# ruolin/strawberry

Measured on AMD Instinct MI355X. Metric: loci/s, EM-to-convergence (+ FPKM/TPM epilogue), C3, higher is better.
Workload: dtype f64; 1 GPU; C3 human-scale synthetic: 60000 loci/GPU, niso~1+Geom(0.25), nrow~LogNormal(ln30,1), 2e8 fragments; loci_per_gpu=60000, fragments_per_gpu=200000086, collective=none (one rank), steps_pipelined=True

## Files before the change

### strawberry_amd/csrc/sbgpu_api.hip

```cpp
#include <hip/hip_runtime.h>

#include <cstdio>
#include <cstdlib>
#include <chrono>
#include <cmath>
#include <cstring>
#include <mutex>
#include <new>
#include <string>
#include <system_error>
#include <thread>
#include <vector>

#include "../../include/sbgpu.h"
#include "api_internal.h"
#include "binweight_device.h"
#include "em_device.h"
#include "em_wide.h"
#include "plan.h"

namespace {

thread_local std::string g_err;

int fail(int code, const std::string &msg)
{
   g_err = msg;
   return code;
}

#define HIP_TRY(expr)                                                                         \
   do {                                                                                       \
      hipError_t e_ = (expr);                                                                 \
      if (e_ != hipSuccess)                                                                   \
         return fail(SBGPU_EHIP, std::string(#expr) + ": " + hipGetErrorString(e_));          \
   } while (0)

constexpr int kAuxStreams = 8;
constexpr int kMaxPhaseEvents = 6;
constexpr int kKindStream[sb::kNumKinds] = {0, 0, 0, 2, 6, 1};

}

struct sbgpu_ctx {
   int device = 0;
   int n_cu = 256;
   hipDeviceProp_t prop;
   hipStream_t stream = nullptr;
   hipStream_t aux[kAuxStreams] = {};
   hipEvent_t fork = nullptr;
   hipEvent_t join[kAuxStreams] = {};
   unsigned split_runs = 0;
   int wave_alt = -1;
   hipEvent_t t0[sb::kNumKinds] = {}, t1[sb::kNumKinds] = {};
   hipEvent_t tp[kMaxPhaseEvents + 1] = {};
   bool timed[sb::kNumKinds] = {};
   bool timing = false;
   int n_phase_timed = 0;
   char *scratch[sb::kScratchSlots] = {};
   size_t scratch_bytes[sb::kScratchSlots] = {};
   int32_t *d_pdf_support = nullptr;
   int32_t *wide_error = nullptr;
   static constexpr int kMaxStages = 16;
   hipEvent_t stage_ev[kMaxStages][2] = {};
   const char *stage_name[kMaxStages] = {};
   int n_stages = 0;
   bool stage_open = false;
   char *pinned[4] = {};
   size_t pinned_bytes[4] = {};
   hipStream_t copy_stream = nullptr;
   hipEvent_t order_ev[6] = {};
   size_t pairs_hint = 0;
   sb::ResidentAnnotation *resident = nullptr;
   sb::ContextKeep context_keep;
   char *boot_scratch = nullptr;
   size_t boot_scratch_cap = 0;
   sb::BootKeep boot_keep;
   char *boot_result = nullptr;
   size_t boot_result_cap = 0;
};

namespace sb {
int api_fail(int code, const std::string &msg) { return fail(code, msg); }
hipStream_t ctx_stream(const sbgpu_ctx_t *ctx) { return ctx->stream; }
hipStream_t ctx_aux_stream(const sbgpu_ctx_t *ctx, int i) { return (i >= 0 && i < kAuxStreams) ? ctx->aux[i] : ctx->stream; }
int ctx_cu_count(const sbgpu_ctx_t *ctx) { return ctx->n_cu; }
int ctx_device(const sbgpu_ctx_t *ctx) { return ctx->device; }
void ctx_stage_reset(sbgpu_ctx_t *ctx) { ctx->n_stages = 0, ctx->stage_open = false; }
void ctx_stage_begin(sbgpu_ctx_t *ctx, const char *name, hipStream_t s)
{
   if (!ctx->timing || ctx->stage_open || ctx->n_stages >= sbgpu_ctx::kMaxStages) return;
   hipEvent_t *ev = ctx->stage_ev[ctx->n_stages];
   for (int i = 0; i < 2; ++i)
      if (!ev[i] && hipEventCreate(&ev[i]) != hipSuccess) return;
   if (hipEventRecord(ev[0], s) != hipSuccess) return;
   ctx->stage_name[ctx->n_stages] = name;
   ctx->stage_open = true;
}
void ctx_stage_end(sbgpu_ctx_t *ctx, hipStream_t s)
{
   if (!ctx->stage_open) return;
   (void)hipEventRecord(ctx->stage_ev[ctx->n_stages][1], s);
   ctx->stage_open = false;
   ++ctx->n_stages;
}
hipError_t ctx_pinned(sbgpu_ctx_t *ctx, int slot, size_t bytes, char **out)
{
   *out = nullptr;
   if (slot < 0 || slot >= 4) return hipErrorInvalidValue;
   if (bytes < 4096) bytes = 4096;
   if (ctx->pinned_bytes[slot] < bytes) {
      if (ctx->pinned[slot]) (void)hipHostFree(ctx->pinned[slot]);
      ctx->pinned[slot] = nullptr;
      ctx->pinned_bytes[slot] = 0;
      const size_t want = bytes + bytes / 4;
      hipError_t e = hipHostMalloc((void **)&ctx->pinned[slot], want, hipHostMallocDefault);
      if (e != hipSuccess) return e;
      ctx->pinned_bytes[slot] = want;
   }
   *out = ctx->pinned[slot];
   return hipSuccess;
}
hipError_t ctx_copy_stream(sbgpu_ctx_t *ctx, hipStream_t *out)
{
   if (!ctx->copy_stream) {
      hipError_t e = hipStreamCreateWithFlags(&ctx->copy_stream, hipStreamNonBlocking);
      if (e != hipSuccess) return e;
   }
   *out = ctx->copy_stream;
   return hipSuccess;
}
hipError_t ctx_event(sbgpu_ctx_t *ctx, int which, hipEvent_t *out)
{
   if (which < 0 || which >= 6) return hipErrorInvalidValue;
   if (!ctx->order_ev[which]) {
      hipError_t e = hipEventCreateWithFlags(&ctx->order_ev[which], hipEventDisableTiming);
      if (e != hipSuccess) return e;
   }
   *out = ctx->order_ev[which];
   return hipSuccess;
}
namespace {
struct DevBlock {
   char *p;
   size_t cap;
   int device;
};
struct DevPool {
   std::mutex m;
   std::vector<DevBlock> blocks;
   size_t bytes = 0;
   size_t limit = 0;
};
size_t dev_pool_limit(DevPool &pool)
{
   if (pool.limit) return pool.limit;
   size_t lim = (size_t)4 << 30;
   if (const char *e = std::getenv("SBGPU_POOL_GB")) {
      lim = (size_t)std::max(0.0, std::atof(e) * 1073741824.0);
   } else {
      size_t free_b = 0, total_b = 0;
      if (hipMemGetInfo(&free_b, &total_b) == hipSuccess && total_b / 2 > lim) lim = total_b / 2;
      else (void)hipGetLastError();
   }
   pool.limit = lim ? lim : 1;
   return pool.limit;
}
DevPool &dev_pool()
{
   static DevPool *p = new DevPool();
   return *p;
}
}
hipError_t dev_take(size_t bytes, char **out, size_t *capacity)
{
   *out = nullptr;
   *capacity = 0;
   if (bytes < 256) bytes = 256;
   int device = 0;
   hipError_t e = hipGetDevice(&device);
   if (e != hipSuccess) return e;
   DevPool &pool = dev_pool();
   {
      std::lock_guard<std::mutex> g(pool.m);
      size_t best = pool.blocks.size();
      for (size_t i = 0; i < pool.blocks.size(); ++i) {
         const DevBlock &b = pool.blocks[i];
         if (b.device == device && b.cap >= bytes && b.cap <= 2 * bytes + (1u << 20) && (best == pool.blocks.size() || b.cap < pool.blocks[best].cap)) best = i;
      }
      if (best < pool.blocks.size()) {
         *out = pool.blocks[best].p;
         *capacity = pool.blocks[best].cap;
         pool.bytes -= pool.blocks[best].cap;
         pool.blocks.erase(pool.blocks.begin() + (long)best);
         return hipSuccess;
      }
   }
   const size_t want = bytes + bytes / 16;
   e = hipMalloc(out, want);
   if (e != hipSuccess) {
      std::vector<DevBlock> idle;
      {
         std::lock_guard<std::mutex> g(pool.m);
         idle.swap(pool.blocks);
         pool.bytes = 0;
      }
      for (const DevBlock &b : idle) (void)hipFree(b.p);
      (void)hipGetLastError();
      e = hipMalloc(out, want);
      if (e != hipSuccess) return e;
   }
   *capacity = want;
   return hipSuccess;
}
size_t dev_release_idle()
{
   std::vector<DevBlock> idle;
   size_t bytes = 0;
   {
      DevPool &pool = dev_pool();
      std::lock_guard<std::mutex> g(pool.m);
      idle.swap(pool.blocks);
      bytes = pool.bytes;
      pool.bytes = 0;
   }
   for (const DevBlock &b : idle) (void)hipFree(b.p);
   return bytes;
}
namespace {
thread_local int g_give_without_device_sync = 0;
}
DevGiveStreamSynced::DevGiveStreamSynced() { ++g_give_without_device_sync; }
DevGiveStreamSynced::~DevGiveStreamSynced() { --g_give_without_device_sync; }
void dev_give(char *block, size_t capacity)
{
   if (!block) return;
   int current = 0, owner = -1;
   const bool have_current = hipGetDevice(&current) == hipSuccess;
// ... 188 lines not shown
            if (kb < 0) {
               k = 2;
            } else {
               kb = 1e3 / kb;
            }
         } else {
            kb = 1e3 / (double)len[u];
         }
         if (k != 2) {
            f = th[u] * rpm * kb;
            sum_fpkm += f;
         }
         fpkm[jb + u] = f;
         keep[jb + u] = k;
      }
   }
   double kept_sum = 0.0;
   for (int64_t jb = j0; jb < j1; jb += 4) {
      double f[4];
      int32_t kk[4];
#pragma unroll
      for (int u = 0; u < 4; ++u) {
         const bool in = jb + u < j1;
         f[u] = in ? fpkm[jb + u] : 0.0;
         kk[u] = in ? keep[jb + u] : 0;
      }
#pragma unroll
      for (int u = 0; u < 4; ++u) {
         if (jb + u >= j1) break;
         double fr = 0.0;
         int32_t k = kk[u];
         if (k != 2) fr = f[u] / sum_fpkm;
         if (p.filter_by_expression && fr < p.min_isoform_frac) k = 0;
         frac[jb + u] = fr;
         keep[jb + u] = k;
         if (k) kept_sum += f[u];
      }
   }
   return kept_sum;
}

__global__ __launch_bounds__(256) void abundance_kernel(int64_t n_loci, const int64_t *iso_off, const double *theta,
                                                        const int32_t *status, const int32_t *length,
                                                        sbgpu_abundance_params_t p, double *fpkm, double *frac,
                                                        int32_t *keep, double *block_sum, unsigned *ticket, double *total)
{
   const int64_t l = (int64_t)blockIdx.x * blockDim.x + threadIdx.x;
   __shared__ double part[256];
   __shared__ int s_last;
   part[threadIdx.x] = l < n_loci ? abundance_locus(l, iso_off, theta, status, length, p, fpkm, frac, keep) : 0.0;
   __syncthreads();
   for (int w = 128; w > 0; w >>= 1) {
      if ((int)threadIdx.x < w) part[threadIdx.x] += part[threadIdx.x + w];
      __syncthreads();
   }
   if (threadIdx.x == 0) {
      __hip_atomic_store(&block_sum[blockIdx.x], part[0], __ATOMIC_RELAXED, __HIP_MEMORY_SCOPE_AGENT);
      asm volatile("s_waitcnt vmcnt(0)" ::: "memory");
      const unsigned t = __hip_atomic_fetch_add(ticket, 1u, __ATOMIC_RELAXED, __HIP_MEMORY_SCOPE_AGENT);
      s_last = t == gridDim.x - 1;
   }
   __syncthreads();
   if (!s_last) return;
   double acc = 0.0;
   for (unsigned i = threadIdx.x; i < gridDim.x; i += 256)
      acc += __hip_atomic_load(&block_sum[i], __ATOMIC_RELAXED, __HIP_MEMORY_SCOPE_AGENT);
   part[threadIdx.x] = acc;
   __syncthreads();
   for (int w = 128; w > 0; w >>= 1) {
      if ((int)threadIdx.x < w) part[threadIdx.x] += part[threadIdx.x + w];
      __syncthreads();
   }
   if (threadIdx.x == 0) {
      *total = part[0];
      __hip_atomic_store(ticket, 0u, __ATOMIC_RELAXED, __HIP_MEMORY_SCOPE_AGENT);
   }
}

__global__ __launch_bounds__(1024) void sum_kernel(int64_t n, const double *x, double *out)
{
   __shared__ double s[1024];
   double acc = 0.0;
   for (int64_t i = threadIdx.x; i < n; i += 1024) acc += x[i];
   s[threadIdx.x] = acc;
   __syncthreads();
   for (int w = 512; w > 0; w >>= 1) {
      if ((int)threadIdx.x < w) s[threadIdx.x] += s[threadIdx.x + w];
      __syncthreads();
   }
   if (threadIdx.x == 0) *out = s[0];
}

__global__ void delay_kernel(unsigned long long ticks)
{
   const unsigned long long t0 = __builtin_amdgcn_s_memrealtime();
   while (__builtin_amdgcn_s_memrealtime() - t0 < ticks) __builtin_amdgcn_s_sleep(32);
}

__global__ void tpm_kernel(int64_t n, const double *fpkm, const int32_t *keep, const double *total,
                           double *tpm)
{
   const int64_t i = (int64_t)blockIdx.x * blockDim.x + threadIdx.x;
   if (i >= n) return;
   const double t = *total;
   tpm[i] = keep[i] ? 1e6 * fpkm[i] / t : 0.0;
}

}

extern "C" {

const char *sbgpu_version(void) { return "libsbgpu 0.1 (gfx950, strawberry EM hot path)"; }

#ifndef SBGPU_BUILD_ID
#define SBGPU_BUILD_ID "unknown"
#endif
const char *sbgpu_build_id(void) { return SBGPU_BUILD_ID; }

const char *sbgpu_last_error(void) { return g_err.c_str(); }

int sbgpu_device_count(void)
{
   int n = 0;
   if (hipGetDeviceCount(&n) != hipSuccess) return 0;
   return n;
}

int sbgpu_init(int device, sbgpu_ctx_t **ctx_out)
{
   if (!ctx_out) return fail(SBGPU_EINVAL, "sbgpu_init: null ctx_out");
   *ctx_out = nullptr;
   int n = 0;
   if (hipGetDeviceCount(&n) != hipSuccess || n <= 0) return fail(SBGPU_ENODEV, "sbgpu_init: no HIP device");
   if (device < 0 || device >= n) return fail(SBGPU_ENODEV, "sbgpu_init: device index out of range");
   HIP_TRY(hipSetDevice(device));
   sbgpu_ctx *c = new (std::nothrow) sbgpu_ctx();
   if (!c) return fail(SBGPU_ENOMEM, "sbgpu_init: out of host memory");
   c->device = device;
   hipError_t e = hipGetDeviceProperties(&c->prop, device);
   if (e != hipSuccess) {
      delete c;
      return fail(SBGPU_EHIP, std::string("hipGetDeviceProperties: ") + hipGetErrorString(e));
   }
   if (std::strncmp(c->prop.gcnArchName, "gfx950", 6) != 0) {
      std::string arch = c->prop.gcnArchName;
      delete c;
      return fail(SBGPU_ENODEV, "sbgpu_init: device is " + arch + ", libsbgpu is built for gfx950 only");
   }
   c->n_cu = c->prop.multiProcessorCount;
   e = hipStreamCreateWithFlags(&c->stream, hipStreamNonBlocking);
   int prio_least = 0, prio_greatest = 0;
   (void)hipDeviceGetStreamPriorityRange(&prio_least, &prio_greatest);
   const bool use_prio = !(sb::exp_env("SBGPU_STREAM_PRIORITY") && std::atoi(sb::exp_env("SBGPU_STREAM_PRIORITY")) == 0);
   for (int i = 0; e == hipSuccess && i < kAuxStreams; ++i) {
      const bool long_kind = i == kKindStream[sb::kNumKinds - 1] || i == kKindStream[sb::kNumKinds - 2] || i == kKindStream[sb::kNumKinds - 3];
      e = hipStreamCreateWithPriority(&c->aux[i], hipStreamNonBlocking, (use_prio && long_kind) ? prio_greatest : 0);
      if (e == hipSuccess) e = hipEventCreateWithFlags(&c->join[i], hipEventDisableTiming);
   }
   if (e == hipSuccess) e = hipEventCreateWithFlags(&c->fork, hipEventDisableTiming);
   if (e == hipSuccess) e = hipMalloc((void **)&c->d_pdf_support, 8 * sizeof(int32_t));
   if (e == hipSuccess) e = hipHostMalloc((void **)&c->wide_error, sizeof(int32_t), hipHostMallocDefault);
   if (e == hipSuccess) *c->wide_error = 0;
   for (int k = 0; e == hipSuccess && k < sb::kNumKinds; ++k) {
      e = hipEventCreate(&c->t0[k]);
      if (e == hipSuccess) e = hipEventCreate(&c->t1[k]);
   }
   for (int i = 0; e == hipSuccess && i <= kMaxPhaseEvents; ++i) e = hipEventCreate(&c->tp[i]);
   if (e != hipSuccess) {
      sbgpu_finalize(c);
      return fail(SBGPU_EHIP, std::string("sbgpu_init: stream/event creation: ") + hipGetErrorString(e));
   }
   *ctx_out = c;
   return SBGPU_OK;
}

int sbgpu_finalize(sbgpu_ctx_t *c)
{
   if (!c) return SBGPU_OK;
   (void)hipSetDevice(c->device);
   for (int i = 0; i < kAuxStreams; ++i) {
      if (c->aux[i]) (void)hipStreamDestroy(c->aux[i]);
      if (c->join[i]) (void)hipEventDestroy(c->join[i]);
   }
   if (c->fork) (void)hipEventDestroy(c->fork);
   for (int k = 0; k < sb::kNumKinds; ++k) {
      if (c->t0[k]) (void)hipEventDestroy(c->t0[k]);
      if (c->t1[k]) (void)hipEventDestroy(c->t1[k]);
   }
   for (int i = 0; i <= kMaxPhaseEvents; ++i)
      if (c->tp[i]) (void)hipEventDestroy(c->tp[i]);
   if (c->stream) (void)hipStreamDestroy(c->stream);
   if (c->wide_error) (void)hipHostFree(c->wide_error);
   for (auto &ev : c->stage_ev)
      for (hipEvent_t e : ev)
         if (e) (void)hipEventDestroy(e);
   if (c->d_pdf_support) (void)hipFree(c->d_pdf_support);
   for (int i = 0; i < sb::kScratchSlots; ++i)
      if (c->scratch[i]) (void)hipFree(c->scratch[i]);
   for (int i = 0; i < 4; ++i)
      if (c->pinned[i]) (void)hipHostFree(c->pinned[i]);
   for (hipEvent_t ev : c->order_ev)
      if (ev) (void)hipEventDestroy(ev);
   if (c->copy_stream) (void)hipStreamDestroy(c->copy_stream);
   sb::ctx_boot_release(c);
   sb::ctx_set_resident_annotation(c, nullptr);
   sb::dev_give(c->boot_scratch, c->boot_scratch_cap);
   delete c;
   return SBGPU_OK;
}

int sbgpu_device_info(sbgpu_ctx_t *c, int64_t out[8])
{
   if (!c || !out) return fail(SBGPU_EINVAL, "sbgpu_device_info: null argument");
   out[0] = c->prop.multiProcessorCount;
   out[1] = c->prop.warpSize;
   out[2] = (int64_t)c->prop.maxSharedMemoryPerMultiProcessor;
   out[3] = c->prop.clockRate;
   out[4] = (int64_t)(c->prop.totalGlobalMem >> 20);
   out[5] = out[6] = out[7] = 0;
   return SBGPU_OK;
}

int64_t sbgpu_release_idle_memory(void) { return (int64_t)sb::dev_release_idle(); }

int sbgpu_synchronize(sbgpu_ctx_t *c, void *stream)
{
   if (!c) return fail(SBGPU_EINVAL, "sbgpu_synchronize: null ctx");
   HIP_TRY(hipStreamSynchronize((hipStream_t)stream));
   if (c->wide_error && *c->wide_error) {
      *c->wide_error = 0;
      return fail(SBGPU_EHIP, "a barrier of the wide-locus EM kernel timed out: the loci it served have no result");
   }
   return SBGPU_OK;
}

int sbgpu_plan_destroy(sbgpu_plan_t *p)
{
   if (!p) return SBGPU_OK;
   if (p->ctx) (void)hipSetDevice(p->ctx->device);
   sb::dev_give(p->d_arena, p->arena_cap);
   if (p->graph_exec) (void)hipGraphExecDestroy(p->graph_exec);
   delete p;
   return SBGPU_OK;
}

int sbgpu_plan_create(sbgpu_ctx_t *c, int64_t n_loci, const int64_t *row_off, const int64_t *iso_off,
                      const int64_t *f_off, sbgpu_plan_t **plan_out)
{
   if (!c || !plan_out) return fail(SBGPU_EINVAL, "sbgpu_plan_create: null argument");
   *plan_out = nullptr;
   sbgpu_plan *p = new (std::nothrow) sbgpu_plan();
   if (!p) return fail(SBGPU_ENOMEM, "sbgpu_plan_create: out of host memory");
   p->ctx = c;
   const char *err = "";
   sb::PlanTuning tune;
   if (const char *e = sb::exp_env("SBGPU_WAVE_RMULT")) tune.wave_rmult = std::atoi(e);
   if (const char *e = sb::exp_env("SBGPU_MAX_WAVES")) tune.max_waves = std::atoll(e);
   if (const char *e = sb::exp_env("SBGPU_LIGHT_BLOCK")) tune.light_block = std::atoi(e) != 0;
   if (const char *e = sb::exp_env("SBGPU_ORDER")) tune.order_by_work = std::string(e) == "work";
   if (const char *e = sb::exp_env("SBGPU_CLASS_ORDER")) tune.classes_by_prediction = std::string(e) != "cost";
   auto parse_list = [](const char *ev, auto conv, auto *out) {
      std::string spec = ev;
      size_t pos = 0;
      while (pos < spec.size()) {
         size_t q = spec.find(',', pos);
         if (q == std::string::npos) q = spec.size();
         out->push_back(conv(spec.substr(pos, q - pos)));
         pos = q + 1;
      }
   };
   if (const char *e = sb::exp_env("SBGPU_PHASES")) {
      tune.phases_auto = false;
      parse_list(e, [](const std::string &t) { return std::atoi(t.c_str()); }, &tune.phase_limits);
   }
   if (const char *e = sb::exp_env("SBGPU_PHASE_LAMBDA"))
      parse_list(e, [](const std::string &t) { return (!t.empty() && (t[0] == 't' || t[0] == 'T')) ? -1.0 : std::atof(t.c_str()); }, &tune.phase_lambda);
   const bool timing = std::getenv("SBGPU_HOST_TIMING") != nullptr;
   auto now = []() { return std::chrono::duration<double>(std::chrono::steady_clock::now().time_since_epoch()).count(); };
   double t_stage = now();
   auto stage = [&](const char *name) {
      if (timing) {
         const double t = now();
         std::fprintf(stderr, "sbgpu_plan_create: %-12s %.2f ms\n", name, (t - t_stage) * 1e3);
         t_stage = t;
      }
   };
   int rc = sb::build_host_plan(n_loci, row_off, iso_off, f_off, c->n_cu, tune, &p->host, &err);
   stage("size classes");
   if (rc != SBGPU_OK) {
      delete p;
      return fail(rc, err);
   }
   if (n_loci > 0) p->h_row_off.assign(row_off, row_off + n_loci + 1), p->h_iso_off.assign(iso_off, iso_off + n_loci + 1);
   else p->h_row_off.assign(1, 0), p->h_iso_off.assign(1, 0);
   auto bail = [&](hipError_t e, const char *what) {
      sbgpu_plan_destroy(p);
      return fail(e == hipErrorOutOfMemory ? SBGPU_ENOMEM : SBGPU_EHIP, std::string(what) + ": " + hipGetErrorString(e));
   };
   hipError_t e = hipSetDevice(c->device);
   if (e != hipSuccess) return bail(e, "hipSetDevice");
   const size_t nb = (size_t)(n_loci + 1) * sizeof(int64_t);
   std::vector<sb::WideDesc> wide_table;
   size_t wide_buf_doubles = 0;
   for (sb::SizeClass &sc : p->host.classes) {
      if (sc.kind != sb::kStream) continue;
      std::vector<std::pair<int, int32_t>> wide;
      std::vector<int32_t> rest;
// ... 66 lines not shown
      for (int32_t cap : p->host.lat[0].capacity) n_phased += cap;
   auto up = [](size_t bytes) { return (bytes + 255) & ~(size_t)255; };
   size_t at = 0;
   const size_t o_row = at; at += up(nb);
   const size_t o_iso = at; at += up(nb);
   const size_t o_f = at; at += up(nb);
   const size_t o_loci = at; at += up((size_t)(n_loci + 1) * sizeof(int32_t));
   const size_t o_tab = at; at += up(ncls_alloc * sizeof(sb::ClassDesc));
   const size_t o_cn = at; at += up(ncls_alloc * sizeof(int32_t));
   const size_t o_wtab = at; at += up((wide_table.size() + 1) * sizeof(sb::WideDesc));
   std::vector<size_t> o_ltab(nlat), o_lroute(nlat), o_lcnt(nlat), o_ltot(nlat), o_llist(nlat);
   for (size_t i = 0; i < nlat; ++i) {
      o_ltab[i] = at; at += up((p->host.lat[i].classes.size() + 1) * sizeof(sb::ClassDesc));
      o_lroute[i] = at; at += up((size_t)(n_loci + 1) * sizeof(int32_t));
   }
   const size_t o_tick = at; at += up(sizeof(unsigned));
   const size_t staged = at;
   const size_t o_cur = at;
   for (size_t i = 0; i < nlat; ++i) {
      o_lcnt[i] = at; at += up((p->host.lat[i].classes.size() + 1) * sizeof(int32_t));
      o_ltot[i] = at; at += up(sizeof(int32_t));
   }
   p->zero_bytes = at - o_cur;
   for (size_t i = 0; i < nlat; ++i) {
      o_llist[i] = at; at += up((size_t)(n_phased + 1) * sizeof(int32_t));
   }
   const size_t o_keep = at; at += up((size_t)p->host.n_rows + 1);
   const size_t o_sum = at; at += up((size_t)(n_loci + 1) * sizeof(double));
   const size_t o_wbuf = at; at += up((wide_buf_doubles + 1) * sizeof(double));
   if ((e = sb::dev_take(at, &p->d_arena, &p->arena_cap)) != hipSuccess) return bail(e, "hipMalloc(plan arena)");
   stage("hipMalloc");
   p->d_row_off = (int64_t *)(p->d_arena + o_row);
   p->d_iso_off = (int64_t *)(p->d_arena + o_iso);
   p->d_f_off = (int64_t *)(p->d_arena + o_f);
   p->d_loci_all = (int32_t *)(p->d_arena + o_loci);
   p->d_tables = (sb::ClassDesc *)(p->d_arena + o_tab);
   p->d_class_n = (int32_t *)(p->d_arena + o_cn);
   p->d_zero = p->d_arena + o_cur;
   p->lat.resize(nlat);
   for (size_t i = 0; i < nlat; ++i) {
      sbgpu_plan::LatDev &ld = p->lat[i];
      const sb::LatPhase &lp = p->host.lat[i];
      ld.d_table = (sb::ClassDesc *)(p->d_arena + o_ltab[i]);
      ld.d_route = (int32_t *)(p->d_arena + o_lroute[i]);
      ld.d_counts = (int32_t *)(p->d_arena + o_lcnt[i]);
      ld.d_total = (int32_t *)(p->d_arena + o_ltot[i]);
      ld.d_lists = (int32_t *)(p->d_arena + o_llist[i]);
      ld.n_classes = (int)lp.classes.size();
      ld.it_limit = lp.it_limit;
      ld.repack = lp.repack;
      ld.grid = (int)std::min<int64_t>(std::max<int64_t>(lp.max_blocks, 1), 32768);
   }
   p->d_row_keep = (uint8_t *)(p->d_arena + o_keep);
   p->d_locus_sum = (double *)(p->d_arena + o_sum);
   p->d_epi_ticket = (unsigned *)(p->d_arena + o_tick);
   p->d_wide_table = (sb::WideDesc *)(p->d_arena + o_wtab);
   p->d_wide_bufs = (double *)(p->d_arena + o_wbuf);
   std::vector<char> stage_buf(staged, 0);
   if (n_loci > 0) {
      std::memcpy(stage_buf.data() + o_row, row_off, nb);
      std::memcpy(stage_buf.data() + o_iso, iso_off, nb);
      std::memcpy(stage_buf.data() + o_f, f_off, nb);
   }
   int32_t *h_loci = (int32_t *)(stage_buf.data() + o_loci);
   sb::ClassDesc *table = (sb::ClassDesc *)(stage_buf.data() + o_tab);
   int32_t *h_cn = (int32_t *)(stage_buf.data() + o_cn);
   if (!wide_table.empty()) std::memcpy(stage_buf.data() + o_wtab, wide_table.data(), wide_table.size() * sizeof(sb::WideDesc));
   for (size_t i = 0; i < nlat; ++i) {
      const sb::LatPhase &lp = p->host.lat[i];
      sb::ClassDesc *lt = (sb::ClassDesc *)(stage_buf.data() + o_ltab[i]);
      int32_t loff = 0;
      for (size_t ci = 0; ci < lp.classes.size(); ++ci) {
         const sb::SizeClass &sc = lp.classes[ci];
         lt[ci].block_begin = 0;
         lt[ci].n = lp.capacity[ci];
         lt[ci].loci_off = loff;
         lt[ci].shape = sc.layout | (sc.rmult << 8) | (sc.lbG << 16);
         loff += lp.capacity[ci];
      }
      std::memcpy(stage_buf.data() + o_lroute[i], lp.route.data(), lp.route.size() * sizeof(int32_t));
   }
   size_t off = 0;
   size_t max_stream_iso = 0;
   for (int k = 0; k < sb::kNumKinds; ++k) p->launches[k] = KindLaunch();
   for (size_t ci = 0; ci < ncls; ++ci) {
      const sb::SizeClass &sc = p->host.classes[ci];
      KindLaunch &kl = p->launches[sc.kind];
      if (kl.n_classes == 0) {
         kl.first_class = (int)ci;
         kl.d_table = p->d_tables + ci;
         kl.block_threads = sc.block_threads;
      }
      table[ci].block_begin = kl.n_blocks;
      table[ci].n = (int32_t)sc.loci.size();
      table[ci].loci_off = (int32_t)off;
      table[ci].shape = sc.layout | (sc.rmult << 8) | (sc.lbG << 16);
      h_cn[ci] = table[ci].n;
      kl.n_blocks += sc.n_blocks;
      kl.n_classes += 1;
      std::memcpy(h_loci + off, sc.loci.data(), sc.loci.size() * sizeof(int32_t));
      p->loci_off.push_back((int64_t)off);
      off += sc.loci.size();
      if (sc.kind == sb::kStream) {
         for (int32_t l : sc.loci) {
            size_t k = (size_t)(iso_off[l + 1] - iso_off[l]);
            if (k > max_stream_iso) max_stream_iso = k;
         }
      }
   }
   stage("staging");
   if ((e = hipMemcpy(p->d_arena, stage_buf.data(), staged, hipMemcpyHostToDevice)) != hipSuccess) return bail(e, "hipMemcpy(plan)");
   if (wide_buf_doubles && (e = hipMemset(p->d_wide_bufs, 0, wide_buf_doubles * sizeof(double))) != hipSuccess) return bail(e, "hipMemset(plan)");
   stage("upload");
   size_t npad = 1;
   while (npad < max_stream_iso && npad < 64) npad <<= 1;
   if (max_stream_iso > 64) npad = 64 * ((max_stream_iso + 63) / 64);
   p->stream_lds_bytes = (3 + sb::kStreamThreads / 64) * npad * sizeof(double);
   *plan_out = p;
   return SBGPU_OK;
}

int sbgpu_plan_info(const sbgpu_plan_t *p, int64_t out[8])
{
   if (!p || !out) return fail(SBGPU_EINVAL, "sbgpu_plan_info: null argument");
   out[0] = p->host.n_loci;
   out[1] = p->host.n_rows;
   out[2] = p->host.n_iso;
   out[3] = p->host.n_elem;
   out[4] = (int64_t)p->host.classes.size();
   out[5] = p->host.n_stream_loci;
   out[6] = p->host.algorithmic_bytes;
   out[7] = p->n_wide_loci;
   return SBGPU_OK;
}

int sbgpu_plan_classes(const sbgpu_plan_t *p, int64_t *out, int cap)
{
   if (!p) return fail(SBGPU_EINVAL, "sbgpu_plan_classes: null plan");
   int n = (int)p->host.classes.size();
   for (int i = 0; i < n && i < cap && out; ++i) {
      const sb::SizeClass &sc = p->host.classes[i];
      out[i * 6 + 0] = sc.kind;
      out[i * 6 + 1] = sc.CPL * sc.CL;
      out[i * 6 + 2] = sc.R;
      out[i * 6 + 3] = sc.G;
      out[i * 6 + 4] = (int64_t)sc.loci.size();
      out[i * 6 + 5] = (int64_t)sc.n_blocks * (sc.block_threads / 64);
   }
   return n;
}

}

static int find_wave_alt(sbgpu_ctx_t *c)
{
   const int used[3] = {kKindStream[sb::kWaveH], kKindStream[sb::kBlock], kKindStream[sb::kBlockTall]};
   const int cand[5] = {1, 3, 4, 5, 7};
   if (hipDeviceSynchronize() != hipSuccess) return 0;
   for (int pass = 0; pass < 2; ++pass)
      for (int ci = 0; ci < 5; ++ci) {
         const auto t0 = std::chrono::steady_clock::now();
         for (int u = 0; u < 3; ++u) hipLaunchKernelGGL(delay_kernel, dim3(1), dim3(64), 0, c->aux[used[u]], 200ull * 100ull);
         hipLaunchKernelGGL(delay_kernel, dim3(1), dim3(64), 0, c->aux[cand[ci]], 200ull * 100ull);
         if (hipDeviceSynchronize() != hipSuccess) return 0;
         const double us = std::chrono::duration<double, std::micro>(std::chrono::steady_clock::now() - t0).count();
         if (pass == 1 && us < 330.0) return cand[ci];
      }
   return 0;
}

static int em_run_impl(sbgpu_ctx_t *c, const sbgpu_plan_t *p, const int32_t *d_count, const void *d_F_any, void *d_theta_any,
                       int32_t *d_status, int32_t *d_iters, void *stream, const bool f32, const void *d_row_bias = nullptr,
                       const void *d_iso_bias = nullptr, void *join_stream = nullptr)
{
   if (!c || !p) return fail(SBGPU_EINVAL, "sbgpu_em_run_device: null ctx/plan");
   if (p->host.n_loci == 0) return SBGPU_OK;
   if (!d_theta_any || !d_status || !d_iters || (!d_count && p->host.n_rows) || (!d_F_any && p->host.n_elem))
      return fail(SBGPU_EINVAL, "sbgpu_em_run_device: null device pointer");
   if (f32 && (p->launches[sb::kStream].n_classes > 0 || p->launches[sb::kWaveH].n_classes > 0))
      return fail(SBGPU_EUNSUPPORTED, "sbgpu_em_run_device_f32: the fp32 variant covers loci of up to 64 isoforms in the tile kernels only");
   if ((d_row_bias != nullptr) != (d_iso_bias != nullptr)) return fail(SBGPU_EINVAL, "sbgpu_em_run_device_bias: both bias arrays or none");
   bool stream_fallback = false;
   if (p->launches[sb::kStream].n_classes > 0)
      stream_fallback = (int32_t)p->host.classes[p->launches[sb::kStream].first_class].loci.size() > p->n_wide_loci;
   if (d_row_bias && (stream_fallback || !p->lat.empty()))
      return fail(SBGPU_EUNSUPPORTED, "sbgpu_em_run_device_bias: the bias factors are applied at tile load (tile kernels and the wide-locus kernel: "
                                      "no locus on the streaming fallback, no phases)");
   hipStream_t main = (hipStream_t)stream;
   sb::EmArgs a;
   a.row_bias = f32 ? nullptr : (const double *)d_row_bias;
   a.iso_bias = f32 ? nullptr : (const double *)d_iso_bias;
   a.row_off = p->d_row_off;
   a.iso_off = p->d_iso_off;
   a.f_off = p->d_f_off;
   a.count = d_count;
   a.F = (const double *)d_F_any;
   a.theta = (double *)d_theta_any;
   a.status = d_status;
   a.iters = d_iters;
   sb::EmArgsT<float> a32;
   a32.row_off = a.row_off, a32.iso_off = a.iso_off, a32.f_off = a.f_off, a32.count = a.count;
   a32.F = (const float *)d_F_any, a32.theta = (float *)d_theta_any, a32.status = d_status, a32.iters = d_iters;
   a32.row_bias = f32 ? (const float *)d_row_bias : nullptr, a32.iso_bias = f32 ? (const float *)d_iso_bias : nullptr;
   if (join_stream && (p->zero_bytes || p->n_wide_desc))
      for (int k = 0; k < sb::kNumKinds; ++k)
         if (p->launches[k].n_classes > 0) HIP_TRY(hipStreamWaitEvent(main, c->join[k], 0));
   if (p->zero_bytes) HIP_TRY(hipMemsetAsync(p->d_zero, 0, p->zero_bytes, main));
   if (p->n_wide_desc) HIP_TRY(hipMemsetAsync(d_status, 0xFF, (size_t)p->host.n_loci * sizeof(int32_t), main));
   int kinds = 0;
   for (int k = 0; k < sb::kNumKinds; ++k) kinds += p->launches[k].n_classes > 0;
   const bool fork = kinds > 1;
   static const bool wave_on_main = sb::exp_env("SBGPU_WAVE_ON_MAIN") && std::atoi(sb::exp_env("SBGPU_WAVE_ON_MAIN")) != 0;
   if (join_stream && fork && c->wave_alt < 0) {
      const char *forced = sb::exp_env("SBGPU_WAVE_ALT");
      c->wave_alt = forced ? std::max(0, std::min(7, std::atoi(forced))) : find_wave_alt(c);
      if (std::getenv("SBGPU_HOST_TIMING"))
         std::fprintf(stderr, "[sbgpu] split runs: the wave kinds' second stream = %d (0: none)%s\n", c->wave_alt, forced ? " (SBGPU_WAVE_ALT)" : "");
   }
   const int wave_slot = (join_stream && fork && c->wave_alt > 0 && !p->zero_bytes && !p->n_wide_desc && (c->split_runs++ & 1)) ? c->wave_alt : 0;
   auto stream_of = [&](int k) -> hipStream_t {
      if (!fork || (wave_on_main && kKindStream[k] == 0)) return main;
      return c->aux[kKindStream[k] == 0 ? wave_slot : kKindStream[k]];
   };
   if (fork) {
      HIP_TRY(hipEventRecord(c->fork, main));
      for (int k = 0; k < sb::kNumKinds; ++k)
         if (p->launches[k].n_classes > 0 && stream_of(k) != main) HIP_TRY(hipStreamWaitEvent(stream_of(k), c->fork, 0));
   }
   for (int k = 0; k < sb::kNumKinds; ++k) c->timed[k] = false;
   c->n_phase_timed = 0;
   const bool timing = c->timing;
   const bool wide_last = fork && p->n_wide_desc > 0;
   for (int pass = 0; pass < 2; ++pass)
   for (int k = sb::kNumKinds - 1; k >= 0; --k) {
      const KindLaunch &kl = p->launches[k];
      if (kl.n_classes == 0) continue;
      if ((pass == 1) != (wide_last && k == sb::kStream)) continue;
      if (pass == 1) {
         for (int o = 0; o < sb::kNumKinds; ++o) {
            if (o == k || p->launches[o].n_classes == 0) continue;
            HIP_TRY(hipEventRecord(c->join[o], stream_of(o)));
            HIP_TRY(hipStreamWaitEvent(stream_of(k), c->join[o], 0));
         }
      }
      hipStream_t s = stream_of(k);
      static const int wave_delay_us = sb::exp_env("SBGPU_WAVE_DELAY_US") ? std::atoi(sb::exp_env("SBGPU_WAVE_DELAY_US")) : 5;
      static const int block_delay_us = sb::exp_env("SBGPU_BLOCK_DELAY_US") ? std::atoi(sb::exp_env("SBGPU_BLOCK_DELAY_US")) : 5;
      const bool tall_runs = p->launches[sb::kBlockTall].n_classes > 0;
      int hold_us = 0;
      if (fork && k == sb::kBlock && tall_runs) hold_us = block_delay_us;
      if (fork && kKindStream[k] == 0) hold_us = wave_delay_us + ((tall_runs && p->launches[sb::kBlock].n_classes > 0) ? block_delay_us : 0);
      if (join_stream && !(p->zero_bytes || p->n_wide_desc)) hold_us = 0;
      if (hold_us > 0) {
         hipLaunchKernelGGL(delay_kernel, dim3(1), dim3(64), 0, s, (unsigned long long)hold_us * 100ull);
         HIP_TRY(hipGetLastError());
      }
      if (timing) HIP_TRY(hipEventRecord(c->t0[k], s));
      if (k == sb::kStream) {
         if (p->n_wide_desc) {
            p->wide_epoch = (p->wide_epoch % 0x1FFFFFu) + 1;
            int32_t *d_err = nullptr;
            HIP_TRY(hipHostGetDevicePointer((void **)&d_err, c->wide_error, 0));
            for (const sbgpu_plan::WideRound &r : p->wide_rounds) {
               sb::WideArgs wa;
               wa.a = a;
               wa.table = p->d_wide_table + r.first_desc;
               wa.n_desc = r.n_desc;
               wa.bufs = p->d_wide_bufs;
               wa.epoch = p->wide_epoch;
               wa.error = d_err;
               HIP_TRY(sb::launch_wide(wa, r.n_blocks, r.lds_bytes, s));
            }
         }
         const int32_t n_all = (int32_t)p->host.classes[kl.first_class].loci.size();
         if (n_all > p->n_wide_loci) {
            sb::ClassArgs ca = {};
            ca.loci = p->d_loci_all + p->loci_off[kl.first_class] + p->n_wide_loci;
            ca.n = n_all - p->n_wide_loci;
            ca.batch = 0;
            HIP_TRY(sb::launch_stream(a, ca, p->d_row_keep, ca.n, p->stream_lds_bytes, s));
         }
      } else {
         const bool wave_kind = k == sb::kWaveH || k == sb::kWave1 || k == sb::kWave2;
         const bool phased = wave_kind && !p->lat.empty() && !f32;
         sb::FusedLaunch fl;
         fl.a = a;
         fl.ph.table = kl.d_table;
         fl.ph.n_classes = kl.n_classes;
         fl.ph.lists_in = p->d_loci_all;
         fl.ph.n_in = p->d_class_n + kl.first_class;
         fl.ph.n_batches = kl.n_blocks;
         fl.ph.total_blocks = nullptr;
         fl.ph.lists_out = phased ? p->lat[0].d_lists : nullptr;
         fl.ph.n_out = phased ? p->lat[0].d_counts : nullptr;
         fl.ph.route = phased ? p->lat[0].d_route : nullptr;
         fl.ph.next_table = phased ? p->lat[0].d_table : nullptr;
         fl.ph.it_limit = phased ? p->host.first_limit : SBGPU_EM_MAX_ITER;
         fl.ph.resume = 0;
         fl.n_blocks = std::max(1, (int)(kl.n_blocks * p->host.grid_scale + 0.5));
         hipError_t e = hipErrorInvalidValue;
         if (f32) {
            sb::FusedLaunchF32 f;
            f.a = a32, f.ph = fl.ph, f.n_blocks = fl.n_blocks;
            e = sb::launch_fused_f32(k, f, s);
         } else if (k == sb::kWaveH) e = sb::launch_fused_wave_h(fl, s);
         else if (k == sb::kWave1) e = sb::launch_fused_wave_1(fl, s);
         else if (k == sb::kWave2) e = sb::launch_fused_wave_2(fl, s);
         else if (k == sb::kBlock) e = sb::launch_fused_block(fl, s);
         else if (k == sb::kBlockTall) e = sb::launch_fused_block_tall(fl, s);
         HIP_TRY(e);
         for (size_t i = 0; phased && i < p->lat.size(); ++i) {
            const sbgpu_plan::LatDev &ld = p->lat[i];
            const bool last = i + 1 == p->lat.size();
            if (timing && i < (size_t)kMaxPhaseEvents) HIP_TRY(hipEventRecord(c->tp[i], s));
            HIP_TRY(sb::launch_phase_prepare(ld.d_table, ld.d_counts, ld.n_classes, ld.d_total, s));
            sb::FusedLaunch ll;
            ll.a = a;
            ll.ph.table = ld.d_table;
            ll.ph.n_classes = ld.n_classes;
            ll.ph.lists_in = ld.d_lists;
            ll.ph.n_in = ld.d_counts;
            ll.ph.n_batches = 0;
            ll.ph.total_blocks = ld.d_total;
            ll.ph.lists_out = last ? nullptr : p->lat[i + 1].d_lists;
            ll.ph.n_out = last ? nullptr : p->lat[i + 1].d_counts;
            ll.ph.route = last ? nullptr : p->lat[i + 1].d_route;
            ll.ph.next_table = last ? nullptr : p->lat[i + 1].d_table;
            ll.ph.it_limit = ld.it_limit;
            ll.ph.resume = 1;
            ll.n_blocks = ld.grid;
            hipError_t el = hipErrorInvalidValue;
            if (!ld.repack) el = sb::launch_lat(ll, s);
            else if (k == sb::kWaveH) el = sb::launch_fused_wave_h(ll, s);
            else if (k == sb::kWave1) el = sb::launch_fused_wave_1(ll, s);
            else el = sb::launch_fused_wave_2(ll, s);
            HIP_TRY(el);
            if (timing) c->n_phase_timed = (int)std::min<size_t>(i + 1, kMaxPhaseEvents);
         }
         if (timing && phased && p->lat.size() <= (size_t)kMaxPhaseEvents) HIP_TRY(hipEventRecord(c->tp[p->lat.size()], s));
      }
      if (timing) {
         HIP_TRY(hipEventRecord(c->t1[k], s));
         c->timed[k] = true;
      }
   }
   hipStream_t join_to = join_stream ? (hipStream_t)join_stream : main;
   if (fork) {
      for (int k = 0; k < sb::kNumKinds; ++k) {
         if (p->launches[k].n_classes == 0) continue;
         if (stream_of(k) == join_to) continue;
         HIP_TRY(hipEventRecord(c->join[k], stream_of(k)));
         HIP_TRY(hipStreamWaitEvent(join_to, c->join[k], 0));
      }
   } else if (join_to != main) {
      HIP_TRY(hipEventRecord(c->fork, main));
      HIP_TRY(hipStreamWaitEvent(join_to, c->fork, 0));
   }
   return SBGPU_OK;
}

extern "C" {

int sbgpu_em_run_device(sbgpu_ctx_t *c, const sbgpu_plan_t *p, const int32_t *d_count, const double *d_F,
                        double *d_theta, int32_t *d_status, int32_t *d_iters, void *stream)
{
   static const bool use_graph = sb::exp_env("SBGPU_GRAPH") && std::atoi(sb::exp_env("SBGPU_GRAPH")) != 0;
   if (!use_graph || !c || !p || c->timing || p->n_wide_desc)
      return em_run_impl(c, p, d_count, d_F, d_theta, d_status, d_iters, stream, false);
   const void *key[6] = {d_count, d_F, d_theta, d_status, d_iters, stream};
   if (!p->graph_exec || std::memcmp(key, p->graph_key, sizeof key) != 0) {
      if (p->graph_exec) (void)hipGraphExecDestroy(p->graph_exec);
      p->graph_exec = nullptr;
      hipGraph_t g = nullptr;
      HIP_TRY(hipStreamBeginCapture(c->stream, hipStreamCaptureModeRelaxed));
      const int rc = em_run_impl(c, p, d_count, d_F, d_theta, d_status, d_iters, c->stream, false);
// ... 463 lines not shown
```

Measured before the change: 89.05 million loci/s.

## Generalize side-stream probe to block kinds and probe via device events

Replaces the wave-only alternate-stream finder with a generic probe that times delay kernels using device events instead of host wall-clock. It also adds optional alternate streams for the block and tall-block kinds, so consecutive runs can alternate queues. Those alternates are off by default (compile-time flags false), so by default only the wave kinds' alternate stream is chosen, now through the new probe. The new probe may pick a different stream than the old one did, which can change overlap between pipelined runs.

```diff
diff --git a/strawberry_amd/csrc/sbgpu_api.hip b/strawberry_amd/csrc/sbgpu_api.hip
--- a/strawberry_amd/csrc/sbgpu_api.hip
+++ b/strawberry_amd/csrc/sbgpu_api.hip
@@ -1,5 +1,6 @@
 #include <hip/hip_runtime.h>
 
+#include <algorithm>
 #include <cstdio>
 #include <cstdlib>
 #include <chrono>
@@ -36,9 +37,12 @@
          return fail(SBGPU_EHIP, std::string(#expr) + ": " + hipGetErrorString(e_));          \
    } while (0)
 
-constexpr int kAuxStreams = 8;
+constexpr int kAuxStreams = 12;
 constexpr int kMaxPhaseEvents = 6;
 constexpr int kKindStream[sb::kNumKinds] = {0, 0, 0, 2, 6, 1};
+constexpr int kBaseStreams = 8;
+constexpr int kAltHigh[2] = {8, 9}, kAltLow[2] = {10, 11};
+constexpr bool kBlockAltDefault = false, kTallAltDefault = false;
 
 }
 
@@ -51,7 +55,9 @@
    hipEvent_t fork = nullptr;
    hipEvent_t join[kAuxStreams] = {};
    unsigned split_runs = 0;
-   int wave_alt = -1;
+   bool alts_known = false;
+   bool told_per_run_state = false;
+   int wave_alt = 0, block_alt = 0, tall_alt = 0;
    hipEvent_t t0[sb::kNumKinds] = {}, t1[sb::kNumKinds] = {};
    hipEvent_t tp[kMaxPhaseEvents + 1] = {};
    bool timed[sb::kNumKinds] = {};
@@ -83,7 +89,7 @@
 namespace sb {
 int api_fail(int code, const std::string &msg) { return fail(code, msg); }
 hipStream_t ctx_stream(const sbgpu_ctx_t *ctx) { return ctx->stream; }
-hipStream_t ctx_aux_stream(const sbgpu_ctx_t *ctx, int i) { return (i >= 0 && i < kAuxStreams) ? ctx->aux[i] : ctx->stream; }
+hipStream_t ctx_aux_stream(const sbgpu_ctx_t *ctx, int i) { return (i >= 0 && i < kBaseStreams) ? ctx->aux[i] : ctx->stream; }
 int ctx_cu_count(const sbgpu_ctx_t *ctx) { return ctx->n_cu; }
 int ctx_device(const sbgpu_ctx_t *ctx) { return ctx->device; }
 void ctx_stage_reset(sbgpu_ctx_t *ctx) { ctx->n_stages = 0, ctx->stage_open = false; }
@@ -578,7 +584,7 @@
    int prio_least = 0, prio_greatest = 0;
    (void)hipDeviceGetStreamPriorityRange(&prio_least, &prio_greatest);
    const bool use_prio = !(sb::exp_env("SBGPU_STREAM_PRIORITY") && std::atoi(sb::exp_env("SBGPU_STREAM_PRIORITY")) == 0);
-   for (int i = 0; e == hipSuccess && i < kAuxStreams; ++i) {
+   for (int i = 0; e == hipSuccess && i < kBaseStreams; ++i) {
       const bool long_kind = i == kKindStream[sb::kNumKinds - 1] || i == kKindStream[sb::kNumKinds - 2] || i == kKindStream[sb::kNumKinds - 3];
       e = hipStreamCreateWithPriority(&c->aux[i], hipStreamNonBlocking, (use_prio && long_kind) ? prio_greatest : 0);
       if (e == hipSuccess) e = hipEventCreateWithFlags(&c->join[i], hipEventDisableTiming);
@@ -951,21 +957,99 @@
 
 }
 
-static int find_wave_alt(sbgpu_ctx_t *c)
-{
-   const int used[3] = {kKindStream[sb::kWaveH], kKindStream[sb::kBlock], kKindStream[sb::kBlockTall]};
-   const int cand[5] = {1, 3, 4, 5, 7};
-   if (hipDeviceSynchronize() != hipSuccess) return 0;
-   for (int pass = 0; pass < 2; ++pass)
-      for (int ci = 0; ci < 5; ++ci) {
-         const auto t0 = std::chrono::steady_clock::now();
-         for (int u = 0; u < 3; ++u) hipLaunchKernelGGL(delay_kernel, dim3(1), dim3(64), 0, c->aux[used[u]], 200ull * 100ull);
-         hipLaunchKernelGGL(delay_kernel, dim3(1), dim3(64), 0, c->aux[cand[ci]], 200ull * 100ull);
-         if (hipDeviceSynchronize() != hipSuccess) return 0;
-         const double us = std::chrono::duration<double, std::micro>(std::chrono::steady_clock::now() - t0).count();
-         if (pass == 1 && us < 330.0) return cand[ci];
-      }
-   return 0;
+static int find_side_stream(sbgpu_ctx_t *c, const int *used, int n_used, const int *cand, int n_cand, const char *what, bool report)
+{
+   constexpr int kMaxUsed = 6;
+   constexpr unsigned long long kHoldTicks = 200ull * 100ull;
+   constexpr float kApartMs = 0.1f;
+   constexpr int kProbeWaitMs = 2000;
+   if (n_used < 1 || n_used > kMaxUsed) return 0;
+   auto is_used = [&](int s) { return std::find(used, used + n_used, s) != used + n_used; };
+   auto wait_for = [&](hipEvent_t ev) {
+      const auto t0 = std::chrono::steady_clock::now();
+      for (;;) {
+         const hipError_t e = hipEventQuery(ev);
+         if (e == hipSuccess) return true;
+         if (e != hipErrorNotReady) return false;
+         if (std::chrono::steady_clock::now() - t0 > std::chrono::milliseconds(kProbeWaitMs)) return false;
+      }
+   };
+   hipEvent_t end[kMaxUsed + 1] = {};
+   bool ok = hipDeviceSynchronize() == hipSuccess;
+   for (int i = 0; ok && i <= n_used; ++i) ok = hipEventCreate(&end[i]) == hipSuccess;
+   for (int i = 0; ok && i < n_used + n_cand; ++i) {
+      const int s = i < n_used ? used[i] : cand[i - n_used];
+      if (s < 0 || s >= kAuxStreams || !c->aux[s] || (i >= n_used && is_used(s))) continue;
+      hipLaunchKernelGGL(delay_kernel, dim3(1), dim3(64), 0, c->aux[s], kHoldTicks);
+      ok = hipGetLastError() == hipSuccess && hipEventRecord(end[0], c->aux[s]) == hipSuccess && wait_for(end[0]);
+   }
+   int found = 0;
+   for (int ci = 0; ok && ci < n_cand && !found; ++ci) {
+      if (cand[ci] <= 0 || cand[ci] >= kAuxStreams || !c->aux[cand[ci]] || is_used(cand[ci])) continue;
+      for (int i = 0; ok && i <= n_used; ++i) {
+         hipStream_t s = c->aux[i < n_used ? used[i] : cand[ci]];
+         hipLaunchKernelGGL(delay_kernel, dim3(1), dim3(64), 0, s, kHoldTicks);
+         ok = hipGetLastError() == hipSuccess && hipEventRecord(end[i], s) == hipSuccess;
+      }
+      for (int i = 0; ok && i <= n_used; ++i) ok = wait_for(end[i]);
+      float apart = 0.f;
+      for (int u = 0; ok && u < n_used; ++u) {
+         float ms = 0.f;
+         ok = hipEventElapsedTime(&ms, end[u], end[n_used]) == hipSuccess;
+         if (std::fabs(ms) > std::fabs(apart)) apart = ms;
+      }
+      if (ok && std::fabs(apart) < kApartMs) found = cand[ci];
+      if (ok && report)
+         std::fprintf(stderr, "[sbgpu] side-stream probe (%s): stream %d ends %+.0f us from the %d streams in use: %s\n", what, cand[ci],
+                      apart * 1e3, n_used, found ? "beside them" : "shares a queue");
+   }
+   for (hipEvent_t ev : end)
+      if (ev) (void)hipEventDestroy(ev);
+   return ok ? found : 0;
+}
+
+static bool create_alt_streams(sbgpu_ctx_t *c)
+{
+   int prio_least = 0, prio_greatest = 0;
+   (void)hipDeviceGetStreamPriorityRange(&prio_least, &prio_greatest);
+   const bool use_prio = !(sb::exp_env("SBGPU_STREAM_PRIORITY") && std::atoi(sb::exp_env("SBGPU_STREAM_PRIORITY")) == 0);
+   for (int i = kBaseStreams; i < kAuxStreams; ++i) {
+      const bool high = i == kAltHigh[0] || i == kAltHigh[1];
+      if (!c->aux[i] && hipStreamCreateWithPriority(&c->aux[i], hipStreamNonBlocking, high ? (use_prio ? prio_greatest : 0) : prio_least) != hipSuccess) {
+         c->aux[i] = nullptr;
+         return false;
+      }
+   }
+   return true;
+}
+
+static void find_kind_alts(sbgpu_ctx_t *c)
+{
+   const bool report = std::getenv("SBGPU_HOST_TIMING") != nullptr;
+   const char *forced[3] = {sb::exp_env("SBGPU_WAVE_ALT"), sb::exp_env("SBGPU_BLOCK_ALT"), sb::exp_env("SBGPU_TALL_ALT")};
+   const bool alt_streams = (forced[0] || forced[1] || forced[2] || kBlockAltDefault || kTallAltDefault) && create_alt_streams(c);
+   const int n_streams = alt_streams ? kAuxStreams : kBaseStreams;
+   const bool by_default[3] = {true, kBlockAltDefault && alt_streams, kTallAltDefault && alt_streams};
+   const char *what[3] = {"wave kinds", "block kind", "tall block kind"};
+   const int cand[3][5] = {{1, 3, 4, 5, 7},
+                           {kAltHigh[0], kKindStream[sb::kStream], kAltLow[0], 0, 0},
+                           {kAltHigh[1], kKindStream[sb::kStream], kAltLow[1], 0, 0}};
+   const int n_cand[3] = {5, 3, 3};
+   int used[6] = {kKindStream[sb::kWaveH], kKindStream[sb::kBlock], kKindStream[sb::kBlockTall]}, n_used = 3;
+   int *slot[3] = {&c->wave_alt, &c->block_alt, &c->tall_alt};
+   bool pinned[3];
+   for (int i = 0; i < 3; ++i) {
+      pinned[i] = forced[i] && std::atoi(forced[i]) >= 0;
+      if (pinned[i]) *slot[i] = std::min(n_streams - 1, std::atoi(forced[i]));
+      else *slot[i] = (forced[i] || by_default[i]) ? find_side_stream(c, used, n_used, cand[i], n_cand[i], what[i], report) : 0;
+      if (*slot[i] > 0 && std::find(used, used + n_used, *slot[i]) == used + n_used) used[n_used++] = *slot[i];
+   }
+   c->alts_known = true;
+   if (report) {
+      std::fprintf(stderr, "[sbgpu] split runs: the wave kinds' second stream = %d (0: none)%s\n", c->wave_alt, pinned[0] ? " (SBGPU_WAVE_ALT)" : "");
+      std::fprintf(stderr, "[sbgpu] split runs: second streams of the block kind = %d, of the tall block kind = %d (0: none)%s%s\n", c->block_alt,
+                   c->tall_alt, pinned[1] ? " (SBGPU_BLOCK_ALT)" : "", pinned[2] ? " (SBGPU_TALL_ALT)" : "");
+   }
 }
 
 static int em_run_impl(sbgpu_ctx_t *c, const sbgpu_plan_t *p, const int32_t *d_count, const void *d_F_any, void *d_theta_any,
@@ -1010,16 +1094,25 @@
    for (int k = 0; k < sb::kNumKinds; ++k) kinds += p->launches[k].n_classes > 0;
    const bool fork = kinds > 1;
    static const bool wave_on_main = sb::exp_env("SBGPU_WAVE_ON_MAIN") && std::atoi(sb::exp_env("SBGPU_WAVE_ON_MAIN")) != 0;
-   if (join_stream && fork && c->wave_alt < 0) {
-      const char *forced = sb::exp_env("SBGPU_WAVE_ALT");
-      c->wave_alt = forced ? std::max(0, std::min(7, std::atoi(forced))) : find_wave_alt(c);
+   if (join_stream && fork && !c->alts_known) find_kind_alts(c);
+   const bool odd_run = join_stream && fork && !p->zero_bytes && !p->n_wide_desc && (c->split_runs++ & 1);
+   if (join_stream && fork && (p->zero_bytes || p->n_wide_desc) && !c->told_per_run_state) {
+      c->told_per_run_state = true;
       if (std::getenv("SBGPU_HOST_TIMING"))
-         std::fprintf(stderr, "[sbgpu] split runs: the wave kinds' second stream = %d (0: none)%s\n", c->wave_alt, forced ? " (SBGPU_WAVE_ALT)" : "");
-   }
-   const int wave_slot = (join_stream && fork && c->wave_alt > 0 && !p->zero_bytes && !p->n_wide_desc && (c->split_runs++ & 1)) ? c->wave_alt : 0;
+         std::fprintf(stderr, "[sbgpu] split runs: a plan with per-run state (phases, wide loci) alternates no kind: its runs wait for each other\n");
+   }
+   const bool stream_kind_runs = p->launches[sb::kStream].n_classes > 0;
+   auto slot_of = [&](int k) -> int {
+      int alt = 0;
+      if (kKindStream[k] == 0) alt = c->wave_alt;
+      else if (k == sb::kBlock) alt = c->block_alt;
+      else if (k == sb::kBlockTall) alt = c->tall_alt;
+      if (kKindStream[k] != 0 && alt == kKindStream[sb::kStream] && stream_kind_runs) alt = 0;
+      return (odd_run && alt > 0) ? alt : kKindStream[k];
+   };
    auto stream_of = [&](int k) -> hipStream_t {
       if (!fork || (wave_on_main && kKindStream[k] == 0)) return main;
-      return c->aux[kKindStream[k] == 0 ? wave_slot : kKindStream[k]];
+      return c->aux[slot_of(k)];
    };
    if (fork) {
       HIP_TRY(hipEventRecord(c->fork, main));
```

Result: no change. 88.69 million loci/s (-0.4%).
